# worldlife123/cbench_BaSIC

Hardware: AMD Instinct MI355X
Metric: encode+decode Mpix/s (higher is better)
Workload: dtype f32; 1 GPU; hyperprior codec N=128 M=192 (lossy_graph_scalable_exp_hp), synthetic 3x256x256 images (image i = manual_seed(i), rand), 256 images per GPU per step resident in HBM, compress+decompress incl. bitstream D2H/H2D, 4 concurrent stream workers per GPU (step k on worker k mod W: whole batches, W in flight); images_per_gpu=256, workers=4, rans_waves_per_workgroup=8, batches_in_flight=4, parallelism=image-sharded x1, RCCL all-reduce of metric sums

## Files before the change

### cbench_basic_amd/csrc/conv.hip

```cpp
#include "common.h"

#include <cstdlib>
#include <cstring>
#include <new>
#include <vector>

using namespace basic;

namespace {
thread_local bool g_dynamic_tiles = false;
}
namespace basic {
bool set_dynamic_tiles(bool on)
{
    const bool prev = g_dynamic_tiles;
    g_dynamic_tiles = on;
    return prev;
}
}

namespace {

typedef float f32x16 __attribute__((ext_vector_type(16)));
typedef float f32x4 __attribute__((ext_vector_type(4)));
// ... 337 lines not shown
    if (lane_live && my < g.mh && mx < g.mw && b < g.batch) {
        const int oy = my * g.s_out + g.oy0, ox = mx * g.s_out + g.ox0;
        const int64_t plane = static_cast<int64_t>(g.out_h) * g.out_w;
        float *o = g.out + (static_cast<int64_t>(b) * g.out_ctotal + co_base) * plane + static_cast<int64_t>(oy) * g.out_w + ox;
#pragma unroll
        for (int m = 0; m < MT; ++m)
#pragma unroll
            for (int r = 0; r < 16; ++r) {
                const int co = 32 * m + 8 * (r >> 2) + 4 * khalf + (r & 3);
                if (co < cout_here) {
                    if constexpr (KWB > 0) {
                        f32x2 v2;
                        v2[0] = apply_act(acc[m][r], g.act);
                        v2[1] = apply_act(acc2[m][r], g.act);
                        *reinterpret_cast<f32x2 *>(o + co * plane) = v2;
                    } else {
                        o[co * plane] = apply_act(acc[m][r], g.act);
                    }
                }
            }
    }
}

typedef __bf16 bf16x8 __attribute__((ext_vector_type(8)));
typedef unsigned u32x4 __attribute__((ext_vector_type(4)));

constexpr int kSplitWaves = 8;
constexpr int kSplitThreads = 64 * kSplitWaves;
constexpr int kSplitCK = 16;
constexpr int kSplitStageTaps = 5;
constexpr int kSplitBlockU4 = 4 * 3 * 64;
constexpr int kSplitStageU4 = kSplitStageTaps * kSplitBlockU4;
constexpr int kSplitWSlots = (kSplitStageU4 + kSplitThreads - 1) / kSplitThreads;
static_assert(kSplitWSlots % 2 == 0, "weight stage in two halves");
constexpr size_t kSplitLdsBytes = 2 * kSplitStageU4 * 16 + 2 * 128 * sizeof(float);

__device__ __forceinline__ void split_bf16x3(const float (&x)[8], u32x4 &p0, u32x4 &p1, u32x4 &p2)
{
#pragma unroll
    for (int i = 0; i < 4; ++i) {
        const unsigned a = __float_as_uint(x[2 * i]), b = __float_as_uint(x[2 * i + 1]);
        const unsigned a0 = a & 0xFFFF0000u, b0 = b & 0xFFFF0000u;
        p0[i] = (a >> 16) | b0;
        const unsigned ra = __float_as_uint(x[2 * i] - __uint_as_float(a0)), rb = __float_as_uint(x[2 * i + 1] - __uint_as_float(b0));
        const unsigned a1 = ra & 0xFFFF0000u, b1 = rb & 0xFFFF0000u;
        p1[i] = (ra >> 16) | b1;
        const unsigned sa = __float_as_uint(__uint_as_float(ra) - __uint_as_float(a1)), sb = __float_as_uint(__uint_as_float(rb) - __uint_as_float(b1));
        p2[i] = (sa >> 16) | (sb & 0xFFFF0000u);
    }
}

__device__ __forceinline__ f32x16 mfma_bf16(const u32x4 &a, const u32x4 &b, const f32x16 &c)
{
    return __builtin_amdgcn_mfma_f32_32x32x16_bf16(__builtin_bit_cast(bf16x8, a), __builtin_bit_cast(bf16x8, b), c, 0, 0, 0);
}

constexpr int kSplitPatchPos = 416;
constexpr int kSplitPieceBytes = kSplitPatchPos * 32;
constexpr size_t kSplitLdsPatchBytes = kSplitLdsBytes + 3 * kSplitPieceBytes;
static_assert(kSplitLdsPatchBytes <= 160 * 1024, "patch beside the weight stages");
static_assert(kSplitLdsBytes % 16 == 0, "16-byte aligned patch");
constexpr int kSplitPatchRounds = (2 * kSplitPatchPos + kSplitThreads - 1) / kSplitThreads;

template <int KH, int KW, int KWB, bool PATCH>
__global__ __launch_bounds__(kSplitThreads, 1) void conv_split_bf16_kernel(const TapLaunch g, const u32x4 *wsplit)
{
    constexpr int MT = 4;
    constexpr int kTapsA = KH * KW, kTapsAll = KH * (KW + KWB);
    constexpr int kGroups = kTapsAll / kSplitStageTaps;
    static_assert(kTapsAll % kSplitStageTaps == 0, "taps per channel block must be whole stages");
    static_assert(KWB > 0 && KWB <= KW, "fused phases: second grid inside the first");
    extern __shared__ u32x4 lds_u4[];
    float *chan_const = reinterpret_cast<float *>(lds_u4 + 2 * kSplitStageU4);

    const int tid = threadIdx.x;
    const int lane = tid & 63;
    const int khalf = lane >> 5;
    const int wave = __builtin_amdgcn_readfirstlane(tid >> 6);

    int bid = xcd_tile(blockIdx.x, gridDim.x);
    const int tx_i = bid % g.tiles_x; bid /= g.tiles_x;
    const int ty_i = bid % g.tiles_y; bid /= g.tiles_y;
    const int TB = 1 << g.tb_log, TH = 1 << g.th_log, TW = 1 << g.tw_log;
    const int b0 = bid * TB, my0 = ty_i * TH, mx0 = tx_i * TW;
    struct Pos { int tb, my, mx; };
    auto pos_of = [&](int t) {
        const int qq = (t >> 6) * 32 + (t & 31);
        return Pos{qq >> (g.tw_log + g.th_log), my0 + ((qq >> g.tw_log) & (TH - 1)), mx0 + (qq & (TW - 1))};
    };
    const Pos lp = pos_of(tid);
    const int tb = lp.tb, b = b0 + lp.tb;

    if (tid < 128) {
        chan_const[tid] = g.bias ? g.bias[tid] : 0.f;
        chan_const[128 + tid] = g.beta ? g.beta[tid] : 1.f;
    }

    const int64_t plane = static_cast<int64_t>(g.in_h) * g.in_w;
    const int nimg = (g.batch - b0 < TB) ? g.batch - b0 : TB;
    const __amdgpu_buffer_rsrc_t rsrc = __builtin_amdgcn_make_buffer_rsrc(
        const_cast<float *>(g.in + static_cast<int64_t>(b0) * g.cin * plane), 0, static_cast<int>(nimg * g.cin * plane * 4), 0x00020000);
    const int gy_l = lp.my * g.s_in + g.dymin, gx_l = lp.mx * g.s_in + g.dxmin;
    const int lane_off = static_cast<int>((((static_cast<int64_t>(tb) * g.cin + 8 * khalf) * g.in_h + gy_l) * g.in_w + gx_l) * 4);
    constexpr int kSpanX = KW;
    static_assert(KH * kSpanX <= 32, "one validity bit per tap offset");
    unsigned vmask = 0;
    if (b < g.batch) {
#pragma unroll
        for (int dy = 0; dy < KH; ++dy)
#pragma unroll
            for (int dx = 0; dx < kSpanX; ++dx) {
                const int yy = gy_l + dy, xx = gx_l + dx;
                if (yy >= 0 && yy < g.in_h && xx >= 0 && xx < g.in_w) vmask |= 1u << (dy * kSpanX + dx);
            }
    }
    const int plane_bytes = static_cast<int>(plane * 4);
    auto tap_row = [](int t) { return t < kTapsA ? t / KW : (t - kTapsA) / KWB; };
    auto tap_col = [](int t) { return t < kTapsA ? t % KW : (t - kTapsA) % KWB + (KW - KWB); };
    auto load_b = [&](int cb, int T, float (&d)[8]) __attribute__((always_inline)) {
        const int dy = tap_row(T), dx = tap_col(T);
        const int voff = ((vmask >> (dy * kSpanX + dx)) & 1u) ? lane_off + (dy * g.in_w + dx) * 4 : 0x7FFFFFF0;
        const int soff = cb * kSplitCK * plane_bytes;
#pragma unroll
        for (int j = 0; j < 8; ++j)
            d[j] = __builtin_bit_cast(float, __builtin_amdgcn_raw_buffer_load_b32(rsrc, voff, soff + j * plane_bytes, 0));
    };

    const int ncb = g.cin / kSplitCK;
    constexpr int kHalf = kSplitWSlots / 2;
    u32x4 wst[kHalf];
    auto fetch_w = [&](int s, int h) __attribute__((always_inline)) {
        const u32x4 *src = wsplit + static_cast<int64_t>(s) * kSplitStageU4 + tid;
#pragma unroll
        for (int sl = h * kHalf; sl < (h + 1) * kHalf; ++sl)
            if (sl * kSplitThreads + tid < kSplitStageU4) wst[sl - h * kHalf] = src[sl * kSplitThreads];
    };
    auto store_w = [&](int buf, int h) __attribute__((always_inline)) {
        u32x4 *dst = lds_u4 + buf * kSplitStageU4 + tid;
#pragma unroll
        for (int sl = h * kHalf; sl < (h + 1) * kHalf; ++sl)
            if (sl * kSplitThreads + tid < kSplitStageU4) dst[sl * kSplitThreads] = wst[sl - h * kHalf];
    };

    char *const patch = reinterpret_cast<char *>(lds_u4) + kSplitLdsBytes;
    const int PW = TW + KW - 1, PH = TH + KH - 1, npos = TB * PH * PW;
    int pvoff[kSplitPatchRounds], brow[KH];
    if constexpr (PATCH) {
#pragma unroll
        for (int r = 0; r < kSplitPatchRounds; ++r) {
            const int i = r * kSplitThreads + tid, p = i >> 1, h = i & 1;
            const int prow = p / PW, x = p - prow * PW, img = prow / PH, row = prow - img * PH;
            const int gy = my0 + g.dymin + row, gx = mx0 + g.dxmin + x;
            const bool inside = i < 2 * npos && img < nimg && gy >= 0 && gy < g.in_h && gx >= 0 && gx < g.in_w;
            pvoff[r] = inside ? static_cast<int>((((static_cast<int64_t>(img) * g.cin + 8 * h) * g.in_h + gy) * g.in_w + gx) * 4)
                              : 0x7FFFFFF0;
        }
#pragma unroll
        for (int dy = 0; dy < KH; ++dy) brow[dy] = ((tb * PH + (lp.my - my0) + dy) * PW + (lp.mx - mx0)) * 32 + 16 * khalf;
    }
    float pf[kSplitPatchRounds][8];
    auto fetch_patch = [&](int cb) __attribute__((always_inline)) {
        const int soff = cb * kSplitCK * plane_bytes;
#pragma unroll
        for (int r = 0; r < kSplitPatchRounds; ++r)
#pragma unroll
            for (int j = 0; j < 8; ++j)
                pf[r][j] = __builtin_bit_cast(float, __builtin_amdgcn_raw_buffer_load_b32(rsrc, pvoff[r], soff + j * plane_bytes, 0));
    };
    auto store_patch = [&]() __attribute__((always_inline)) {
#pragma unroll
        for (int r = 0; r < kSplitPatchRounds; ++r)
            if (r * kSplitThreads + tid < 2 * npos) {
                u32x4 q[3];
                split_bf16x3(pf[r], q[0], q[1], q[2]);
#pragma unroll
                for (int pc = 0; pc < 3; ++pc)
                    *reinterpret_cast<u32x4 *>(patch + (r * kSplitThreads + tid) * 16 + pc * kSplitPieceBytes) = q[pc];
            }
    };
    auto read_b = [&](int T, u32x4 (&d)[3]) __attribute__((always_inline)) {
        const char *src = patch + brow[tap_row(T)] + 32 * tap_col(T);
#pragma unroll
        for (int pc = 0; pc < 3; ++pc) d[pc] = *reinterpret_cast<const u32x4 *>(src + pc * kSplitPieceBytes);
    };

    f32x16 acc[MT], acc2[MT];
#pragma unroll
    for (int m = 0; m < MT; ++m)
#pragma unroll
        for (int r = 0; r < 16; ++r) {
            acc[m][r] = 0.f;
            acc2[m][r] = 0.f;
        }

    float xb[8];
    u32x4 bq[2][3];
    if constexpr (PATCH) fetch_patch(0);
    else load_b(0, 0, xb);
    fetch_w(0, 0);
    store_w(0, 0);
    fetch_w(0, 1);
    store_w(0, 1);
    if constexpr (PATCH) store_patch();
    for (int cb = 0; cb < ncb; ++cb) {
#pragma unroll
        for (int gi = 0; gi < kGroups; ++gi) {
            const int s = cb * kGroups + gi;
            __syncthreads();
            const bool more = s + 1 < ncb * kGroups;
            if (more) fetch_w(s + 1, 0);
            __builtin_amdgcn_sched_barrier(0);
            const u32x4 *wl = lds_u4 + (s & 1) * kSplitStageU4 + lane;
#pragma unroll
            for (int tl = 0; tl < kSplitStageTaps; ++tl) {
                const int T = gi * kSplitStageTaps + tl;
                float xn[8];
                u32x4 bd[3];
                if constexpr (PATCH) {
                    if (T == 0) read_b(0, bq[0]);
                } else {
                    if (T + 1 < kTapsAll) load_b(cb, T + 1, xn);
                    else load_b(cb + 1 < ncb ? cb + 1 : cb, 0, xn);
                    __builtin_amdgcn_sched_barrier(0);
                    split_bf16x3(xb, bd[0], bd[1], bd[2]);
                }
                const u32x4 (&bp)[3] = PATCH ? bq[T & 1] : bd;
                f32x16 (&dst)[MT] = T < kTapsA ? acc : acc2;
                u32x4 ap[2][3];
#pragma unroll
                for (int pc = 0; pc < 3; ++pc) ap[0][pc] = wl[(tl * MT * 3 + pc) * 64];
#pragma unroll
                for (int m = 0; m < MT; ++m) {
                    const int cur = m & 1;
                    if (m + 1 < MT) {
#pragma unroll
                        for (int pc = 0; pc < 3; ++pc) ap[cur ^ 1][pc] = wl[((tl * MT + m + 1) * 3 + pc) * 64];
                    } else if constexpr (PATCH) {
                        if (T + 1 < kTapsAll) read_b(T + 1, bq[(T + 1) & 1]);
                    }
                    __builtin_amdgcn_sched_barrier(0);
                    dst[m] = mfma_bf16(ap[cur][2], bp[0], dst[m]);
                    dst[m] = mfma_bf16(ap[cur][1], bp[1], dst[m]);
                    dst[m] = mfma_bf16(ap[cur][0], bp[2], dst[m]);
                    dst[m] = mfma_bf16(ap[cur][1], bp[0], dst[m]);
                    dst[m] = mfma_bf16(ap[cur][0], bp[1], dst[m]);
                    dst[m] = mfma_bf16(ap[cur][0], bp[0], dst[m]);
                    __builtin_amdgcn_sched_barrier(0);
                }
                if constexpr (!PATCH) {
#pragma unroll
                    for (int j = 0; j < 8; ++j) xb[j] = xn[j];
                }
                if (tl == 1 && more) {
                    store_w((s + 1) & 1, 0);
                    fetch_w(s + 1, 1);
                    __builtin_amdgcn_sched_barrier(0);
                }
                if constexpr (PATCH) {
                    if (gi == 0 && tl == 1) {
                        fetch_patch(cb + 1 < ncb ? cb + 1 : cb);
                        __builtin_amdgcn_sched_barrier(0);
                    }
                }
                if (tl == 3 && more) store_w((s + 1) & 1, 1);
            }
        }
        if constexpr (PATCH) {
            if (cb + 1 < ncb) {
                __syncthreads();
                store_patch();
            }
        }
    }

    const int tid_e = wave * 64 + static_cast<int>(__lane_id());
    const int khalf_e = (tid_e >> 5) & 1, col_e = tid_e & 31;
    float *gl = reinterpret_cast<float *>(lds_u4);
    const bool gdn = g.act == BASIC_ACT_GDN || g.act == BASIC_ACT_IGDN;
    auto finish = [&](f32x16 (&acc)[MT]) __attribute__((always_inline)) {
        if (g.bias) {
#pragma unroll
            for (int m = 0; m < MT; ++m)
#pragma unroll
                for (int rq = 0; rq < 4; ++rq) {
                    const f32x4 b4 = *reinterpret_cast<const f32x4 *>(chan_const + 32 * m + 8 * rq + 4 * khalf_e);
#pragma unroll
                    for (int e = 0; e < 4; ++e) acc[m][4 * rq + e] += b4[e];
                }
        }
        if (gdn) {
            f32x16 nrm[MT];
#pragma unroll
            for (int m = 0; m < MT; ++m)
#pragma unroll
                for (int r = 0; r < 16; ++r) nrm[m][r] = 0.f;
#pragma unroll
            for (int st = 0; st < 64; ++st) {
                const int kk = 32 * (st >> 4) + 8 * ((st & 15) >> 2) + (st & 3);
                float gk[4];
                load_a<4>(gl + ((kk + 4 * khalf_e) * 32 + col_e) * 4, gk);
                const float x = acc[st >> 4][st & 15];
                const float bfrag = x * x;
// ... 28 lines not shown

    const Pos ep = pos_of(tid_e);
    const int my = ep.my, mx = ep.mx, be = b0 + ep.tb;
    if (my < g.mh && mx < g.mw && be < g.batch) {
        const int oy = my * g.s_out + g.oy0, ox = mx * g.s_out + g.ox0;
        const int64_t oplane = static_cast<int64_t>(g.out_h) * g.out_w;
        float *o = g.out + (static_cast<int64_t>(be) * g.out_ctotal + g.co_base) * oplane + static_cast<int64_t>(oy) * g.out_w + ox;
#pragma unroll
        for (int m = 0; m < MT; ++m)
#pragma unroll
            for (int r = 0; r < 16; ++r) {
                const int co = 32 * m + 8 * (r >> 2) + 4 * khalf_e + (r & 3);
                if (co < g.cout) {
                    f32x2 v2;
                    v2[0] = apply_act(acc[m][r], g.act);
                    v2[1] = apply_act(acc2[m][r], g.act);
                    *reinterpret_cast<f32x2 *>(o + co * oplane) = v2;
                }
            }
    }
}

template <int KH, bool PATCH>
hipError_t launch_split(const TapLaunch &g, const u32x4 *ws, int blocks, hipStream_t st)
{
    const hipError_t e = ensure_max_lds(reinterpret_cast<const void *>(conv_split_bf16_kernel<KH, 3, 2, PATCH>));
    if (e != hipSuccess) return e;
    hipLaunchKernelGGL((conv_split_bf16_kernel<KH, 3, 2, PATCH>), dim3(blocks), dim3(kSplitThreads),
                       PATCH ? kSplitLdsPatchBytes : kSplitLdsBytes, st, g, ws);
    return hipGetLastError();
}

constexpr int kFirstSlots = 10;

template <bool ROWS>
__global__ __launch_bounds__(512, 1) void conv5x5_cin4_gdn_persistent_kernel(const TapLaunch g, int ntiles, int *sched)
{
    extern __shared__ float lds[];
    constexpr int MT = 4, kCK = ROWS ? 3 : 4, KW = 5, kSteps = ROWS ? 5 * 8 : 25 * 2;
    constexpr int kWFloats = ROWS ? 80 * 32 * 4 : 25 * 4 * 32 * 4;
    constexpr int kGFloats = 128 * 32 * 4;
    float *wl = lds;
    float *gl = lds + kWFloats;
    const int tid = threadIdx.x;
    const int lane = tid & 63;
    const int wave = __builtin_amdgcn_readfirstlane(tid >> 6);
    const int khalf = lane >> 5, col = lane & 31;
    const int TB = 1 << g.tb_log, TH = 1 << g.th_log, TW = 1 << g.tw_log;
    const int chan_stride = g.ph * g.pwp;
    const int patch_elems = TB * kCK * chan_stride;
    const int patch_pad = (patch_elems + 511) / 512 * 512;
    const int n_pslots = patch_pad / 512;
// ... 457 lines not shown
                pr[a][1] = f32x2{mid[0], mid[1]};
                pr[a][2] = f32x2{mid[1], mid[2]};
                pr[a][3] = f32x2{mid[2], mid[3]};
                pr[a][4] = f32x2{mid[3], v5};
            }
            sm_accumulate<STRIPS>(acc, g.wsm + static_cast<int64_t>(c0 + ci) * kSmWRow, pr);
        }
    }
    sm_store<STRIPS>(acc, g, b, my, mx0);
}

struct Phase {
    int ntaps = 0, dymin = 0, dxmin = 0, span_y = 1, span_x = 1;
    int oy0 = 0, ox0 = 0;
    int ck = 2, cin_pad = 0;
    int kh = 0, kw = 0;
    int kwb = 0;
    int waves = 4;
    signed char dy[kMaxTaps], dx[kMaxTaps];
    float *d_wpack = nullptr;
    float *d_wrow = nullptr;
    int64_t split_wstride = 0;
    void *d_wsplit = nullptr;
};

struct Chunk {
    int co0 = 0, cout = 0, coutp = 0, mt = 0;
    int nsplit = 1;
    std::vector<Phase> phases;
    std::vector<Phase> fused;
    float *d_bias = nullptr;
};

}

struct basic_conv_plan {
    int cin = 0, cout = 0, ksize = 0, stride = 1, padding = 0, output_padding = 0, transposed = 0, act = 0;
    int s_in = 1, s_out = 1;
    std::vector<Chunk> chunks;
    std::vector<Chunk> split;
    float *d_gammaT = nullptr, *d_beta = nullptr;
    float *d_wsm = nullptr, *d_bias4 = nullptr;
    int *d_sched = nullptr;
};

extern "C" void basic_conv_plan_destroy(basic_conv_plan *p)
{
    if (!p) return;
    for (auto *list : {&p->chunks, &p->split})
        for (auto &ch : *list) {
            for (auto &ph : ch.phases) {
                if (ph.d_wpack) (void)hipFree(ph.d_wpack);
                if (ph.d_wrow) (void)hipFree(ph.d_wrow);
                if (ph.d_wsplit) (void)hipFree(ph.d_wsplit);
            }
            for (auto &ph : ch.fused) {
                if (ph.d_wpack) (void)hipFree(ph.d_wpack);
                if (ph.d_wsplit) (void)hipFree(ph.d_wsplit);
            }
            if (ch.d_bias) (void)hipFree(ch.d_bias);
        }
    if (p->d_sched) (void)hipFree(p->d_sched);
    if (p->d_wsm) (void)hipFree(p->d_wsm);
    if (p->d_bias4) (void)hipFree(p->d_bias4);
    if (p->d_gammaT) (void)hipFree(p->d_gammaT);
    if (p->d_beta) (void)hipFree(p->d_beta);
    delete p;
}

namespace {

int upload(const std::vector<float> &h, float **d)
{
    BASIC_HIP_TRY(hipMalloc(d, h.size() * sizeof(float)));
    BASIC_HIP_TRY(hipMemcpy(*d, h.data(), h.size() * sizeof(float), hipMemcpyHostToDevice));
    return BASIC_OK;
}

int pack_split(const std::vector<float> &wp, int ck, int ntaps, int cin, void **d)
{
    const int ncb = cin / kSplitCK;
    std::vector<uint16_t> ws(static_cast<size_t>(ncb) * ntaps * kSplitBlockU4 * 8);
    size_t i = 0;
    for (int cb = 0; cb < ncb; ++cb)
        for (int t = 0; t < ntaps; ++t)
            for (int m = 0; m < 4; ++m)
                for (int pc = 0; pc < 3; ++pc)
                    for (int lane = 0; lane < 64; ++lane)
                        for (int j = 0; j < 8; ++j) {
                            const int c = cb * kSplitCK + 8 * (lane >> 5) + j, o = 32 * m + (lane & 31);
                            float rem = wp[((static_cast<size_t>(c / ck) * ntaps + t) * ck + c % ck) * 32 * 4 + (o % 32) * 4 + o / 32];
                            uint32_t u = 0;
                            for (int k = 0; k <= pc; ++k) {
                                std::memcpy(&u, &rem, 4);
                                const uint32_t hi = u & 0xFFFF0000u;
                                float h;
                                std::memcpy(&h, &hi, 4);
                                if (k < pc) rem -= h;
                            }
                            ws[i++] = static_cast<uint16_t>(u >> 16);
                        }
    BASIC_HIP_TRY(hipMalloc(d, ws.size() * sizeof(uint16_t)));
    BASIC_HIP_TRY(hipMemcpy(*d, ws.data(), ws.size() * sizeof(uint16_t), hipMemcpyHostToDevice));
    return BASIC_OK;
}

int build_chunks(basic_conv_plan *p, const float *weight, const float *bias, int cin, int cout, int slice,
                 std::vector<Chunk> *out)
{
    const int ci_n = p->cin, co_n = p->cout, ksize = p->ksize, stride = p->stride, padding = p->padding;
    const bool transposed = p->transposed != 0;
    const int nph = transposed ? stride : 1;
    const int n_chunks = slice ? 1 : (co_n + kMaxCoutPerLaunch - 1) / kMaxCoutPerLaunch;
    const int per_chunk = slice ? co_n : ((co_n + n_chunks - 1) / n_chunks + 31) / 32 * 32;
    const bool gdn = p->act == BASIC_ACT_GDN || p->act == BASIC_ACT_IGDN;
    auto fusable = [](const Phase &a, const Phase &b) {
        return a.ntaps > 0 && b.ntaps > 0 && a.kh == b.kh && a.dymin == b.dymin && b.kw <= a.kw &&
               b.dxmin - a.dxmin == a.kw - b.kw && a.ox0 == 0 && b.ox0 == 1 &&
               ((a.kh == 3 && a.kw == 3 && b.kw == 2) || (a.kh == 2 && a.kw == 3 && b.kw == 2));
    };
    for (int co0 = 0; co0 < co_n; co0 += per_chunk) {
        Chunk ch;
        ch.co0 = co0;
        ch.cout = (co_n - co0 < per_chunk) ? co_n - co0 : per_chunk;
        ch.mt = slice ? slice / 32 : (ch.cout + 31) / 32;
        ch.coutp = ch.mt * 32;
// ... 98 lines not shown
                f.cin_pad = (ci_n + kFusedCK - 1) / kFusedCK * kFusedCK;
                f.d_wpack = nullptr;
                const int mtp = mtile_pitch(ch.mt);
                f.split_wstride = static_cast<int64_t>(f.cin_pad) * f.ntaps * 32 * mtp;
                std::vector<float> wp(static_cast<size_t>(f.split_wstride) * ch.nsplit, 0.f);
                auto tap_weight = [&](int phase_px, int t, int kw_phase, int dymin_p, int dxmin_p, int c, int og) -> float {
                    const int dyv = dymin_p + t / kw_phase, dxv = dxmin_p + t % kw_phase;
                    const int ky = py + padding - dyv * stride, kx = phase_px + padding - dxv * stride;
                    if (ky < 0 || ky >= ksize || kx < 0 || kx >= ksize) return 0.f;
                    return weight[((static_cast<size_t>(c) * cout + og) * ksize + ky) * ksize + kx];
                };
                for (int c = 0; c < ci_n; ++c)
                    for (int t = 0; t < f.ntaps; ++t)
                        for (int o = 0; o < ch.cout; ++o) {
                            const float w = t < a.ntaps ? tap_weight(0, t, a.kw, a.dymin, a.dxmin, c, co0 + o)
                                                        : tap_weight(1, t - a.ntaps, b.kw, b.dymin, b.dxmin, c, co0 + o);
                            const int ol = o % ch.coutp;
                            wp[static_cast<size_t>(o / ch.coutp) * f.split_wstride +
                               (((static_cast<size_t>(c / kFusedCK) * f.ntaps + t) * kFusedCK + (c % kFusedCK)) * 32 + ol % 32) * mtp + ol / 32] = w;
                        }
                wp.resize(wp.size() + kPackTail, 0.f);
                int rcf = upload(wp, &f.d_wpack);
                if (!rcf && !slice && p->act == BASIC_ACT_IGDN && ch.mt == 4 && ch.nsplit == 1 && ci_n % kSplitCK == 0)
                    rcf = pack_split(wp, kFusedCK, f.ntaps, ci_n, &f.d_wsplit);
                fused.push_back(f);
                if (rcf) { ok = false; }
            }
            if (ok) ch.fused = fused;
            else for (auto &f : fused) {
                if (f.d_wpack) (void)hipFree(f.d_wpack);
                if (f.d_wsplit) (void)hipFree(f.d_wsplit);
            }
        }
        std::vector<float> hb(static_cast<size_t>(ch.coutp) * ch.nsplit, 0.f);
        if (bias) std::memcpy(hb.data(), bias + co0, sizeof(float) * ch.cout);
        const int rc = upload(hb, &ch.d_bias);
        out->push_back(ch);
        if (rc) return rc;
    }
    return BASIC_OK;
}

}

extern "C" int basic_conv_plan_create(const float *weight, const float *bias, int cin, int cout, int ksize, int stride,
                                      int padding, int output_padding, int transposed, int activation,
                                      const float *gamma, const float *beta, int cin_active, int cout_active,
                                      basic_conv_plan **out)
{
    BASIC_REQUIRE(weight && out && cin >= 1 && cout >= 1 && ksize >= 1 && ksize <= 5 && stride >= 1 && stride <= 2 &&
                      padding >= 0 && padding <= ksize,
                  "conv_plan_create: unsupported geometry (k<=5, stride<=2)");
    BASIC_REQUIRE(cin_active >= 1 && cin_active <= cin && cout_active >= 1 && cout_active <= cout,
                  "conv_plan_create: active channel slice out of range");
// ... 133 lines not shown
    constexpr int kMany = stage_channels(kMaxTaps, WM), kFew = stage_channels(kFewTaps, WF), kVeryFew = stage_channels(kVeryFewTaps, WV);
    const int inst_ck = g.ntaps > kFewTaps ? kMany : (g.ntaps > kVeryFewTaps ? kFew : kVeryFew);
    BASIC_REQUIRE(inst_ck == plan_ck && plan_waves_ == 4, "conv_forward: plan / kernel instantiation mismatch");
    if (g.ntaps > kFewTaps) {
        if (kh == 5 && kw == 5) return launch_one<MT, kMany, 5, 5, WM>(g, blocks, nsplit, lds_bytes, st);
        return launch_one<MT, kMany, 0, 0, WM>(g, blocks, nsplit, lds_bytes, st);
    }
    if (g.ntaps > kVeryFewTaps) {
        if (kh == 3 && kw == 3) return launch_one<MT, kFew, 3, 3, WF>(g, blocks, nsplit, lds_bytes, st);
        return launch_one<MT, kFew, 0, 0, WF>(g, blocks, nsplit, lds_bytes, st);
    }
    if (kh == 3 && kw == 2) return launch_one<MT, kVeryFew, 3, 2, WV>(g, blocks, nsplit, lds_bytes, st);
    if (kh == 2 && kw == 3) return launch_one<MT, kVeryFew, 2, 3, WV>(g, blocks, nsplit, lds_bytes, st);
    if (kh == 2 && kw == 2) return launch_one<MT, kVeryFew, 2, 2, WV>(g, blocks, nsplit, lds_bytes, st);
    return launch_one<MT, kVeryFew, 0, 0, WV>(g, blocks, nsplit, lds_bytes, st);
}

int ilog2(int v) { int l = 0; while ((1 << (l + 1)) <= v) ++l; return l; }
int pow2_ceil(int v) { int p = 1; while (p < v) p <<= 1; return p; }

}

namespace {
struct LaunchChoice { bool use_split, fuse_ok, bf16x3, split_patch; };
LaunchChoice choose_launches(const basic_conv_plan *p, int batch, int oh, int ow, const void *d_out)
{
    const int64_t pos_blocks = (static_cast<int64_t>(batch) * ((oh + p->s_out - 1) / p->s_out) * ((ow + p->s_out - 1) / p->s_out) + kTilePos - 1) / kTilePos;
    const char *dbg_env = getenv("BASIC_CONV_DEBUG");
    const int dbg = dbg_env ? atoi(dbg_env) : 0;
    LaunchChoice c;
    c.use_split = !p->split.empty() && !(dbg & 8) && (pos_blocks < kSplitBelowBlocks || (dbg & 4));
    c.fuse_ok = ow % 2 == 0 && (reinterpret_cast<uintptr_t>(d_out) & 7) == 0 && !(dbg & 512);
    const char *f32_env = getenv("BASIC_CONV_F32");
    c.bf16x3 = !(f32_env && atoi(f32_env) != 0);
    c.split_patch = !(dbg & 1024);
    return c;
}

template <class F>
int for_each_launch(const basic_conv_plan *p, const LaunchChoice &c, int oh, int ow, F &&fn)
{
    for (const Chunk &ch : (c.use_split ? p->split : p->chunks))
        for (const Phase &ph : ((c.fuse_ok && !ch.fused.empty()) ? ch.fused : ch.phases)) {
            const int mh = (oh - ph.oy0 + p->s_out - 1) / p->s_out, mw = (ow - ph.ox0 + p->s_out - 1) / p->s_out;
            if (mh <= 0 || mw <= 0) continue;
            const int rc = fn(ch, ph, mh, mw);
            if (rc) return rc;
        }
    return BASIC_OK;
}

struct TileShape { int tw, th, tb; };
TileShape tile_shape(int mh, int mw, int tile_pos)
{
    TileShape t;
    t.tw = pow2_ceil(mw); if (t.tw > 16) t.tw = 16;
    t.th = pow2_ceil(mh); if (t.th > tile_pos / t.tw) t.th = tile_pos / t.tw;
// ... 19 lines not shown
    return BASIC_OK;
}
}

extern "C" int basic_conv_plan_launches(const basic_conv_plan *p, int batch, int in_h, int in_w)
{
    int oh = 0, ow = 0;
    if (!p || batch < 1 || basic_conv_plan_out_hw(p, in_h, in_w, &oh, &ow)) return -1;
    if (p->d_wsm) return 1;
    int n = 0;
    for_each_launch(p, choose_launches(p, batch, oh, ow, nullptr), oh, ow, [&](const Chunk &, const Phase &, int, int) { ++n; return BASIC_OK; });
    return n;
}

extern "C" int basic_conv_forward_dev(const basic_conv_plan *p, const float *d_in, int batch, int in_h, int in_w,
                                      float *d_out, void *hip_stream)
{
    BASIC_REQUIRE(p && d_in && d_out && batch >= 1, "conv_forward: bad argument");
    int oh = 0, ow = 0;
    int rc = basic_conv_plan_out_hw(p, in_h, in_w, &oh, &ow);
    if (rc) return rc;
    if (p->d_wsm) return launch_small_deconv(p, d_in, batch, in_h, in_w, d_out, as_stream(hip_stream));
    const LaunchChoice choice = choose_launches(p, batch, oh, ow, d_out);
    return for_each_launch(p, choice, oh, ow, [&](const Chunk &ch, const Phase &ph, int mh, int mw) -> int {
        TapLaunch g{};
        g.in = d_in; g.out = d_out; g.wpack = ph.d_wpack; g.wrow = ph.d_wrow; g.split_wstride = ph.split_wstride; g.bias = ch.d_bias; g.gammaT = p->d_gammaT; g.beta = p->d_beta;
        g.batch = batch; g.cin = p->cin; g.cin_pad = ph.ntaps ? ph.cin_pad : 0; g.cout = ch.cout; g.coutp = ch.coutp; g.out_ctotal = p->cout; g.co_base = ch.co0;
        g.in_h = in_h; g.in_w = in_w; g.out_h = oh; g.out_w = ow;
        g.s_in = p->s_in; g.s_out = p->s_out; g.oy0 = ph.oy0; g.ox0 = ph.ox0;
        g.mh = mh; g.mw = mw;
        g.ntaps = ph.ntaps; g.dymin = ph.dymin; g.dxmin = ph.dxmin;
        std::memcpy(g.dy, ph.dy, sizeof(g.dy));
        std::memcpy(g.dx, ph.dx, sizeof(g.dx));
        g.act = p->act;
        const int kCK = ph.ck;
        if (choice.bf16x3 && ph.d_wsplit) {
            const TileShape ts = tile_shape(g.mh, g.mw, kSplitWaves * 32);
            const int tw = ts.tw, th = ts.th, tb = ts.tb;
            if (static_cast<int64_t>(tb) * p->cin * in_h * in_w * 4 < (1ll << 31)) {
                g.tw_log = ilog2(tw); g.th_log = ilog2(th); g.tb_log = ilog2(tb);
                g.tiles_y = (g.mh + th - 1) / th;
                g.tiles_x = (g.mw + tw - 1) / tw;
                const int blocks = ((batch + tb - 1) / tb) * g.tiles_y * g.tiles_x;
                hipStream_t st = as_stream(hip_stream);
                const u32x4 *ws = static_cast<const u32x4 *>(ph.d_wsplit);
                BASIC_REQUIRE(ph.kw == 3 && ph.kwb == 2 && (ph.kh == 3 || ph.kh == 2), "conv_forward: split-bf16 plan / kernel instantiation mismatch");
                const bool patch = choice.split_patch && g.s_in == 1 && tb * (th + ph.kh - 1) * (tw + ph.kw - 1) <= kSplitPatchPos;
                const hipError_t e = ph.kh == 3 ? (patch ? launch_split<3, true>(g, ws, blocks, st) : launch_split<3, false>(g, ws, blocks, st))
                                                : (patch ? launch_split<2, true>(g, ws, blocks, st) : launch_split<2, false>(g, ws, blocks, st));
                BASIC_HIP_TRY(e);
                return BASIC_OK;
            }
        }
        const int threads = 64 * ph.waves, tile_pos = 32 * ph.waves;
        const TileShape ts = tile_shape(g.mh, g.mw, tile_pos);
        const int tw = ts.tw, th = ts.th;
        int tb = ts.tb;
        const bool first_layer_path = ch.mt == 4 && ch.nsplit == 1 && ph.waves == 8 && ph.kh == 5 && ph.kw == 5 &&
                                      ph.cin_pad == kCK && kCK == 4 && ch.cout == 128 && p->d_gammaT;
        g.ph = (th - 1) * g.s_in + ph.span_y;
        g.pw = (tw - 1) * g.s_in + ph.span_x;
        g.patch4 = (ph.waves == 8 && !first_layer_path && in_w % 4 == 0 && (reinterpret_cast<uintptr_t>(d_in) & 15) == 0) ? 1 : 0;
        g.pwp = g.patch4 ? (g.pw + 3 + 3) / 4 * 4 : (g.pw | 1);
        const int punit = g.patch4 ? 4 : 1;
        const int mtp = mtile_pitch(ch.mt);
        const int wl_floats = g.ntaps * kCK * 32 * mtp, gam_floats = 32 * 32 * mtp;
        const int wl_pad = ((wl_floats > gam_floats ? wl_floats : gam_floats) + 4 * threads - 1) / (4 * threads) * (4 * threads);
        auto patch_slots_needed = [&](int tbv) { return (tbv * kCK * g.ph * g.pwp / punit + threads - 1) / threads; };
        auto lds_need = [&](int tbv) {
            const int patch_pad = ((tbv * kCK * g.ph * g.pwp / punit + 63) & ~63) * punit;
            return sizeof(float) * (2 * static_cast<size_t>(wl_pad + patch_pad) + 32 + 2 * g.coutp);
        };
// ... 58 lines not shown
```

Before: 818.0 Mpix/s.

## Replace bf16x3 split convolution with exponent-scaled fp16x2 split MFMA

The split-precision decoder deconvolution now splits activations and weights into two fp16 pieces instead of three bf16 pieces. That cuts the MFMAs per tile from six to three and shrinks the weight and patch LDS staging by a third. To keep fp16 in range, weights get a per-output-channel power-of-two scale when packed on the host. Activations get a per-image scale taken from a new absmax prepass kernel, and both scales are undone in the epilogue. The cost is an extra read of the input plus a memset, and a single per-plan amax buffer. That buffer is shared across concurrent stream workers and can be reallocated, so there is a race risk. Precision also differs from the three-way bf16 split.

New measurement: 894.2 Mpix/s (median of 6 runs). +9.3%, better.

```diff
diff --git a/cbench_basic_amd/csrc/conv.hip b/cbench_basic_amd/csrc/conv.hip
--- a/cbench_basic_amd/csrc/conv.hip
+++ b/cbench_basic_amd/csrc/conv.hip
@@ -1,5 +1,7 @@
 #include "common.h"
 
+#include <algorithm>
+#include <cmath>
 #include <cstdlib>
 #include <cstring>
 #include <new>
@@ -383,48 +385,76 @@
     }
 }
 
-typedef __bf16 bf16x8 __attribute__((ext_vector_type(8)));
+typedef _Float16 f16x8 __attribute__((ext_vector_type(8)));
+typedef _Float16 f16x2 __attribute__((ext_vector_type(2)));
 typedef unsigned u32x4 __attribute__((ext_vector_type(4)));
+typedef int i32x4 __attribute__((ext_vector_type(4)));
 
 constexpr int kSplitWaves = 8;
 constexpr int kSplitThreads = 64 * kSplitWaves;
 constexpr int kSplitCK = 16;
 constexpr int kSplitStageTaps = 5;
-constexpr int kSplitBlockU4 = 4 * 3 * 64;
+constexpr int kSplitBlockU4 = 4 * 2 * 64;
 constexpr int kSplitStageU4 = kSplitStageTaps * kSplitBlockU4;
 constexpr int kSplitWSlots = (kSplitStageU4 + kSplitThreads - 1) / kSplitThreads;
-static_assert(kSplitWSlots % 2 == 0, "weight stage in two halves");
-constexpr size_t kSplitLdsBytes = 2 * kSplitStageU4 * 16 + 2 * 128 * sizeof(float);
-
-__device__ __forceinline__ void split_bf16x3(const float (&x)[8], u32x4 &p0, u32x4 &p1, u32x4 &p2)
+constexpr size_t kSplitLdsBytes = 2 * kSplitStageU4 * 16 + 3 * 128 * sizeof(float);
+constexpr int kSplitWTop = 13, kSplitXTop = 14;
+
+__device__ __forceinline__ int split_act_exp(unsigned amax_bits)
+{
+    const int e = static_cast<int>(amax_bits >> 23);
+    return (amax_bits == 0 || e >= 255) ? 0 : kSplitXTop + 127 - e;
+}
+
+__device__ __forceinline__ void split_f16x2(const float (&x)[8], int k, u32x4 &p0, u32x4 &p1)
 {
 #pragma unroll
     for (int i = 0; i < 4; ++i) {
-        const unsigned a = __float_as_uint(x[2 * i]), b = __float_as_uint(x[2 * i + 1]);
-        const unsigned a0 = a & 0xFFFF0000u, b0 = b & 0xFFFF0000u;
-        p0[i] = (a >> 16) | b0;
-        const unsigned ra = __float_as_uint(x[2 * i] - __uint_as_float(a0)), rb = __float_as_uint(x[2 * i + 1] - __uint_as_float(b0));
-        const unsigned a1 = ra & 0xFFFF0000u, b1 = rb & 0xFFFF0000u;
-        p1[i] = (ra >> 16) | b1;
-        const unsigned sa = __float_as_uint(__uint_as_float(ra) - __uint_as_float(a1)), sb = __float_as_uint(__uint_as_float(rb) - __uint_as_float(b1));
-        p2[i] = (sa >> 16) | (sb & 0xFFFF0000u);
-    }
-}
-
-__device__ __forceinline__ f32x16 mfma_bf16(const u32x4 &a, const u32x4 &b, const f32x16 &c)
-{
-    return __builtin_amdgcn_mfma_f32_32x32x16_bf16(__builtin_bit_cast(bf16x8, a), __builtin_bit_cast(bf16x8, b), c, 0, 0, 0);
+        f32x2 v;
+        v[0] = __builtin_ldexpf(x[2 * i], k);
+        v[1] = __builtin_ldexpf(x[2 * i + 1], k);
+        const f16x2 h0 = __builtin_convertvector(v, f16x2);
+        const f16x2 h1 = __builtin_convertvector(v - __builtin_convertvector(h0, f32x2), f16x2);
+        p0[i] = __builtin_bit_cast(unsigned, h0);
+        p1[i] = __builtin_bit_cast(unsigned, h1);
+    }
+}
+
+__device__ __forceinline__ f32x16 mfma_f16(const u32x4 &a, const u32x4 &b, const f32x16 &c)
+{
+    return __builtin_amdgcn_mfma_f32_32x32x16_f16(__builtin_bit_cast(f16x8, a), __builtin_bit_cast(f16x8, b), c, 0, 0, 0);
+}
+
+__global__ __launch_bounds__(256) void image_absmax_kernel(const float *x, int64_t n, int per_img, unsigned *amax)
+{
+    const int img = blockIdx.x / per_img, part = blockIdx.x - img * per_img;
+    const float *src = x + img * n;
+    unsigned m = 0;
+    if (((reinterpret_cast<uintptr_t>(src) | static_cast<uintptr_t>(n * 4)) & 15) == 0) {
+        const u32x4 *s4 = reinterpret_cast<const u32x4 *>(src);
+        for (int64_t i = part * 256 + threadIdx.x; i < n / 4; i += per_img * 256) {
+            const u32x4 v = s4[i];
+#pragma unroll
+            for (int e = 0; e < 4; ++e) m = max(m, v[e] & 0x7FFFFFFFu);
+        }
+    } else {
+        for (int64_t i = part * 256 + threadIdx.x; i < n; i += per_img * 256) m = max(m, __float_as_uint(src[i]) & 0x7FFFFFFFu);
+    }
+#pragma unroll
+    for (int off = 32; off > 0; off >>= 1) m = max(m, static_cast<unsigned>(__shfl_xor(static_cast<int>(m), off)));
+    if ((threadIdx.x & 63) == 0 && m) atomicMax(amax + img, m);
 }
 
 constexpr int kSplitPatchPos = 416;
 constexpr int kSplitPieceBytes = kSplitPatchPos * 32;
-constexpr size_t kSplitLdsPatchBytes = kSplitLdsBytes + 3 * kSplitPieceBytes;
+constexpr size_t kSplitLdsPatchBytes = kSplitLdsBytes + 2 * kSplitPieceBytes;
 static_assert(kSplitLdsPatchBytes <= 160 * 1024, "patch beside the weight stages");
 static_assert(kSplitLdsBytes % 16 == 0, "16-byte aligned patch");
 constexpr int kSplitPatchRounds = (2 * kSplitPatchPos + kSplitThreads - 1) / kSplitThreads;
 
 template <int KH, int KW, int KWB, bool PATCH>
-__global__ __launch_bounds__(kSplitThreads, 1) void conv_split_bf16_kernel(const TapLaunch g, const u32x4 *wsplit)
+__global__ __launch_bounds__(kSplitThreads, 1) void conv_split_f16_kernel(const TapLaunch g, const u32x4 *wsplit, const int *kw,
+                                                                          const unsigned *amax)
 {
     constexpr int MT = 4;
     constexpr int kTapsA = KH * KW, kTapsAll = KH * (KW + KWB);
@@ -455,6 +485,7 @@
     if (tid < 128) {
         chan_const[tid] = g.bias ? g.bias[tid] : 0.f;
         chan_const[128 + tid] = g.beta ? g.beta[tid] : 1.f;
+        reinterpret_cast<int *>(chan_const)[256 + tid] = kw[tid];
     }
 
     const int64_t plane = static_cast<int64_t>(g.in_h) * g.in_w;
@@ -487,25 +518,28 @@
             d[j] = __builtin_bit_cast(float, __builtin_amdgcn_raw_buffer_load_b32(rsrc, voff, soff + j * plane_bytes, 0));
     };
 
+    int kx_l = 0;
+    if constexpr (!PATCH) kx_l = b < g.batch ? split_act_exp(amax[b]) : 0;
+
     const int ncb = g.cin / kSplitCK;
-    constexpr int kHalf = kSplitWSlots / 2;
+    constexpr int kHalf = (kSplitWSlots + 1) / 2;
     u32x4 wst[kHalf];
     auto fetch_w = [&](int s, int h) __attribute__((always_inline)) {
         const u32x4 *src = wsplit + static_cast<int64_t>(s) * kSplitStageU4 + tid;
 #pragma unroll
-        for (int sl = h * kHalf; sl < (h + 1) * kHalf; ++sl)
+        for (int sl = h * kHalf; sl < (h + 1) * kHalf && sl < kSplitWSlots; ++sl)
             if (sl * kSplitThreads + tid < kSplitStageU4) wst[sl - h * kHalf] = src[sl * kSplitThreads];
     };
     auto store_w = [&](int buf, int h) __attribute__((always_inline)) {
         u32x4 *dst = lds_u4 + buf * kSplitStageU4 + tid;
 #pragma unroll
-        for (int sl = h * kHalf; sl < (h + 1) * kHalf; ++sl)
+        for (int sl = h * kHalf; sl < (h + 1) * kHalf && sl < kSplitWSlots; ++sl)
             if (sl * kSplitThreads + tid < kSplitStageU4) dst[sl * kSplitThreads] = wst[sl - h * kHalf];
     };
 
     char *const patch = reinterpret_cast<char *>(lds_u4) + kSplitLdsBytes;
     const int PW = TW + KW - 1, PH = TH + KH - 1, npos = TB * PH * PW;
-    int pvoff[kSplitPatchRounds], brow[KH];
+    int pvoff[kSplitPatchRounds], pkx[kSplitPatchRounds], brow[KH];
     if constexpr (PATCH) {
 #pragma unroll
         for (int r = 0; r < kSplitPatchRounds; ++r) {
@@ -515,6 +549,7 @@
             const bool inside = i < 2 * npos && img < nimg && gy >= 0 && gy < g.in_h && gx >= 0 && gx < g.in_w;
             pvoff[r] = inside ? static_cast<int>((((static_cast<int64_t>(img) * g.cin + 8 * h) * g.in_h + gy) * g.in_w + gx) * 4)
                               : 0x7FFFFFF0;
+            pkx[r] = inside ? split_act_exp(amax[b0 + img]) : 0;
         }
 #pragma unroll
         for (int dy = 0; dy < KH; ++dy) brow[dy] = ((tb * PH + (lp.my - my0) + dy) * PW + (lp.mx - mx0)) * 32 + 16 * khalf;
@@ -532,17 +567,17 @@
 #pragma unroll
         for (int r = 0; r < kSplitPatchRounds; ++r)
             if (r * kSplitThreads + tid < 2 * npos) {
-                u32x4 q[3];
-                split_bf16x3(pf[r], q[0], q[1], q[2]);
-#pragma unroll
-                for (int pc = 0; pc < 3; ++pc)
+                u32x4 q[2];
+                split_f16x2(pf[r], pkx[r], q[0], q[1]);
+#pragma unroll
+                for (int pc = 0; pc < 2; ++pc)
                     *reinterpret_cast<u32x4 *>(patch + (r * kSplitThreads + tid) * 16 + pc * kSplitPieceBytes) = q[pc];
             }
     };
-    auto read_b = [&](int T, u32x4 (&d)[3]) __attribute__((always_inline)) {
+    auto read_b = [&](int T, u32x4 (&d)[2]) __attribute__((always_inline)) {
         const char *src = patch + brow[tap_row(T)] + 32 * tap_col(T);
 #pragma unroll
-        for (int pc = 0; pc < 3; ++pc) d[pc] = *reinterpret_cast<const u32x4 *>(src + pc * kSplitPieceBytes);
+        for (int pc = 0; pc < 2; ++pc) d[pc] = *reinterpret_cast<const u32x4 *>(src + pc * kSplitPieceBytes);
     };
 
     f32x16 acc[MT], acc2[MT];
@@ -555,7 +590,7 @@
         }
 
     float xb[8];
-    u32x4 bq[2][3];
+    u32x4 bq[2][2];
     if constexpr (PATCH) fetch_patch(0);
     else load_b(0, 0, xb);
     fetch_w(0, 0);
@@ -576,36 +611,36 @@
             for (int tl = 0; tl < kSplitStageTaps; ++tl) {
                 const int T = gi * kSplitStageTaps + tl;
                 float xn[8];
-                u32x4 bd[3];
+                u32x4 bd[2];
                 if constexpr (PATCH) {
                     if (T == 0) read_b(0, bq[0]);
                 } else {
                     if (T + 1 < kTapsAll) load_b(cb, T + 1, xn);
                     else load_b(cb + 1 < ncb ? cb + 1 : cb, 0, xn);
                     __builtin_amdgcn_sched_barrier(0);
-                    split_bf16x3(xb, bd[0], bd[1], bd[2]);
-                }
-                const u32x4 (&bp)[3] = PATCH ? bq[T & 1] : bd;
+                    split_f16x2(xb, kx_l, bd[0], bd[1]);
+                }
+                const u32x4 (&bp)[2] = PATCH ? bq[T & 1] : bd;
                 f32x16 (&dst)[MT] = T < kTapsA ? acc : acc2;
-                u32x4 ap[2][3];
-#pragma unroll
-                for (int pc = 0; pc < 3; ++pc) ap[0][pc] = wl[(tl * MT * 3 + pc) * 64];
+                u32x4 ap[3][2];
+#pragma unroll
+                for (int mm = 0; mm < 2; ++mm)
+#pragma unroll
+                    for (int pc = 0; pc < 2; ++pc) ap[mm][pc] = wl[((tl * MT + mm) * 2 + pc) * 64];
 #pragma unroll
                 for (int m = 0; m < MT; ++m) {
-                    const int cur = m & 1;
-                    if (m + 1 < MT) {
-#pragma unroll
-                        for (int pc = 0; pc < 3; ++pc) ap[cur ^ 1][pc] = wl[((tl * MT + m + 1) * 3 + pc) * 64];
-                    } else if constexpr (PATCH) {
-                        if (T + 1 < kTapsAll) read_b(T + 1, bq[(T + 1) & 1]);
+                    const int cur = m % 3;
+                    if (m + 2 < MT) {
+#pragma unroll
+                        for (int pc = 0; pc < 2; ++pc) ap[(m + 2) % 3][pc] = wl[((tl * MT + m + 2) * 2 + pc) * 64];
+                    }
+                    if constexpr (PATCH) {
+                        if (m == MT - 3 && T + 1 < kTapsAll) read_b(T + 1, bq[(T + 1) & 1]);
                     }
                     __builtin_amdgcn_sched_barrier(0);
-                    dst[m] = mfma_bf16(ap[cur][2], bp[0], dst[m]);
-                    dst[m] = mfma_bf16(ap[cur][1], bp[1], dst[m]);
-                    dst[m] = mfma_bf16(ap[cur][0], bp[2], dst[m]);
-                    dst[m] = mfma_bf16(ap[cur][1], bp[0], dst[m]);
-                    dst[m] = mfma_bf16(ap[cur][0], bp[1], dst[m]);
-                    dst[m] = mfma_bf16(ap[cur][0], bp[0], dst[m]);
+                    dst[m] = mfma_f16(ap[cur][1], bp[0], dst[m]);
+                    dst[m] = mfma_f16(ap[cur][0], bp[1], dst[m]);
+                    dst[m] = mfma_f16(ap[cur][0], bp[0], dst[m]);
                     __builtin_amdgcn_sched_barrier(0);
                 }
                 if constexpr (!PATCH) {
@@ -638,7 +673,17 @@
     const int khalf_e = (tid_e >> 5) & 1, col_e = tid_e & 31;
     float *gl = reinterpret_cast<float *>(lds_u4);
     const bool gdn = g.act == BASIC_ACT_GDN || g.act == BASIC_ACT_IGDN;
+    const int be_s = b0 + pos_of(tid_e).tb;
+    const int kx_e = be_s < g.batch ? split_act_exp(amax[be_s]) : 0;
     auto finish = [&](f32x16 (&acc)[MT]) __attribute__((always_inline)) {
+#pragma unroll
+        for (int m = 0; m < MT; ++m)
+#pragma unroll
+            for (int rq = 0; rq < 4; ++rq) {
+                const i32x4 k4 = *reinterpret_cast<const i32x4 *>(chan_const + 256 + 32 * m + 8 * rq + 4 * khalf_e);
+#pragma unroll
+                for (int e = 0; e < 4; ++e) acc[m][4 * rq + e] = __builtin_ldexpf(acc[m][4 * rq + e], -(k4[e] + kx_e));
+            }
         if (g.bias) {
 #pragma unroll
             for (int m = 0; m < MT; ++m)
@@ -713,12 +758,12 @@
 }
 
 template <int KH, bool PATCH>
-hipError_t launch_split(const TapLaunch &g, const u32x4 *ws, int blocks, hipStream_t st)
-{
-    const hipError_t e = ensure_max_lds(reinterpret_cast<const void *>(conv_split_bf16_kernel<KH, 3, 2, PATCH>));
+hipError_t launch_split(const TapLaunch &g, const u32x4 *ws, const int *kw, const unsigned *amax, int blocks, hipStream_t st)
+{
+    const hipError_t e = ensure_max_lds(reinterpret_cast<const void *>(conv_split_f16_kernel<KH, 3, 2, PATCH>));
     if (e != hipSuccess) return e;
-    hipLaunchKernelGGL((conv_split_bf16_kernel<KH, 3, 2, PATCH>), dim3(blocks), dim3(kSplitThreads),
-                       PATCH ? kSplitLdsPatchBytes : kSplitLdsBytes, st, g, ws);
+    hipLaunchKernelGGL((conv_split_f16_kernel<KH, 3, 2, PATCH>), dim3(blocks), dim3(kSplitThreads),
+                       PATCH ? kSplitLdsPatchBytes : kSplitLdsBytes, st, g, ws, kw, amax);
     return hipGetLastError();
 }
 
@@ -1222,6 +1267,7 @@
     float *d_wrow = nullptr;
     int64_t split_wstride = 0;
     void *d_wsplit = nullptr;
+    int *d_wsplit_k = nullptr;
 };
 
 struct Chunk {
@@ -1242,6 +1288,8 @@
     float *d_gammaT = nullptr, *d_beta = nullptr;
     float *d_wsm = nullptr, *d_bias4 = nullptr;
     int *d_sched = nullptr;
+    unsigned *d_amax = nullptr;
+    int amax_cap = 0;
 };
 
 extern "C" void basic_conv_plan_destroy(basic_conv_plan *p)
@@ -1253,14 +1301,17 @@
                 if (ph.d_wpack) (void)hipFree(ph.d_wpack);
                 if (ph.d_wrow) (void)hipFree(ph.d_wrow);
                 if (ph.d_wsplit) (void)hipFree(ph.d_wsplit);
+                if (ph.d_wsplit_k) (void)hipFree(ph.d_wsplit_k);
             }
             for (auto &ph : ch.fused) {
                 if (ph.d_wpack) (void)hipFree(ph.d_wpack);
                 if (ph.d_wsplit) (void)hipFree(ph.d_wsplit);
+                if (ph.d_wsplit_k) (void)hipFree(ph.d_wsplit_k);
             }
             if (ch.d_bias) (void)hipFree(ch.d_bias);
         }
     if (p->d_sched) (void)hipFree(p->d_sched);
+    if (p->d_amax) (void)hipFree(p->d_amax);
     if (p->d_wsm) (void)hipFree(p->d_wsm);
     if (p->d_bias4) (void)hipFree(p->d_bias4);
     if (p->d_gammaT) (void)hipFree(p->d_gammaT);
@@ -1277,31 +1328,38 @@
     return BASIC_OK;
 }
 
-int pack_split(const std::vector<float> &wp, int ck, int ntaps, int cin, void **d)
+int pack_split(const std::vector<float> &wp, int ck, int ntaps, int cin, void **d, int **d_kw)
 {
     const int ncb = cin / kSplitCK;
-    std::vector<uint16_t> ws(static_cast<size_t>(ncb) * ntaps * kSplitBlockU4 * 8);
+    auto w_at = [&](int c, int t, int o) { return wp[((static_cast<size_t>(c / ck) * ntaps + t) * ck + c % ck) * 32 * 4 + (o % 32) * 4 + o / 32]; };
+    std::vector<int> kw(128, 0);
+    for (int o = 0; o < 128; ++o) {
+        float m = 0.f;
+        for (int c = 0; c < cin; ++c)
+            for (int t = 0; t < ntaps; ++t) m = std::fmax(m, std::fabs(w_at(c, t, o)));
+        int e = 0;
+        if (m > 0.f && std::isfinite(m)) {
+            (void)std::frexp(m, &e);
+            kw[o] = kSplitWTop - (e - 1);
+        }
+    }
+    std::vector<_Float16> ws(static_cast<size_t>(ncb) * ntaps * kSplitBlockU4 * 8);
     size_t i = 0;
     for (int cb = 0; cb < ncb; ++cb)
         for (int t = 0; t < ntaps; ++t)
             for (int m = 0; m < 4; ++m)
-                for (int pc = 0; pc < 3; ++pc)
+                for (int pc = 0; pc < 2; ++pc)
                     for (int lane = 0; lane < 64; ++lane)
                         for (int j = 0; j < 8; ++j) {
                             const int c = cb * kSplitCK + 8 * (lane >> 5) + j, o = 32 * m + (lane & 31);
-                            float rem = wp[((static_cast<size_t>(c / ck) * ntaps + t) * ck + c % ck) * 32 * 4 + (o % 32) * 4 + o / 32];
-                            uint32_t u = 0;
-                            for (int k = 0; k <= pc; ++k) {
-                                std::memcpy(&u, &rem, 4);
-                                const uint32_t hi = u & 0xFFFF0000u;
-                                float h;
-                                std::memcpy(&h, &hi, 4);
-                                if (k < pc) rem -= h;
-                            }
-                            ws[i++] = static_cast<uint16_t>(u >> 16);
+                            const float w = std::ldexp(w_at(c, t, o), kw[o]);
+                            const _Float16 w0 = static_cast<_Float16>(w);
+                            ws[i++] = pc ? static_cast<_Float16>(w - static_cast<float>(w0)) : w0;
                         }
-    BASIC_HIP_TRY(hipMalloc(d, ws.size() * sizeof(uint16_t)));
-    BASIC_HIP_TRY(hipMemcpy(*d, ws.data(), ws.size() * sizeof(uint16_t), hipMemcpyHostToDevice));
+    BASIC_HIP_TRY(hipMalloc(d, ws.size() * sizeof(_Float16)));
+    BASIC_HIP_TRY(hipMemcpy(*d, ws.data(), ws.size() * sizeof(_Float16), hipMemcpyHostToDevice));
+    BASIC_HIP_TRY(hipMalloc(d_kw, kw.size() * sizeof(int)));
+    BASIC_HIP_TRY(hipMemcpy(*d_kw, kw.data(), kw.size() * sizeof(int), hipMemcpyHostToDevice));
     return BASIC_OK;
 }
 
@@ -1446,7 +1504,7 @@
                 wp.resize(wp.size() + kPackTail, 0.f);
                 int rcf = upload(wp, &f.d_wpack);
                 if (!rcf && !slice && p->act == BASIC_ACT_IGDN && ch.mt == 4 && ch.nsplit == 1 && ci_n % kSplitCK == 0)
-                    rcf = pack_split(wp, kFusedCK, f.ntaps, ci_n, &f.d_wsplit);
+                    rcf = pack_split(wp, kFusedCK, f.ntaps, ci_n, &f.d_wsplit, &f.d_wsplit_k);
                 fused.push_back(f);
                 if (rcf) { ok = false; }
             }
@@ -1454,6 +1512,7 @@
             else for (auto &f : fused) {
                 if (f.d_wpack) (void)hipFree(f.d_wpack);
                 if (f.d_wsplit) (void)hipFree(f.d_wsplit);
+                if (f.d_wsplit_k) (void)hipFree(f.d_wsplit_k);
             }
         }
         std::vector<float> hb(static_cast<size_t>(ch.coutp) * ch.nsplit, 0.f);
@@ -1633,7 +1692,7 @@
 }
 
 namespace {
-struct LaunchChoice { bool use_split, fuse_ok, bf16x3, split_patch; };
+struct LaunchChoice { bool use_split, fuse_ok, split_f16, split_patch; };
 LaunchChoice choose_launches(const basic_conv_plan *p, int batch, int oh, int ow, const void *d_out)
 {
     const int64_t pos_blocks = (static_cast<int64_t>(batch) * ((oh + p->s_out - 1) / p->s_out) * ((ow + p->s_out - 1) / p->s_out) + kTilePos - 1) / kTilePos;
@@ -1643,7 +1702,7 @@
     c.use_split = !p->split.empty() && !(dbg & 8) && (pos_blocks < kSplitBelowBlocks || (dbg & 4));
     c.fuse_ok = ow % 2 == 0 && (reinterpret_cast<uintptr_t>(d_out) & 7) == 0 && !(dbg & 512);
     const char *f32_env = getenv("BASIC_CONV_F32");
-    c.bf16x3 = !(f32_env && atoi(f32_env) != 0);
+    c.split_f16 =!(f32_env && atoi(f32_env) != 0);
     c.split_patch = !(dbg & 1024);
     return c;
 }
@@ -1709,6 +1768,7 @@
     if (rc) return rc;
     if (p->d_wsm) return launch_small_deconv(p, d_in, batch, in_h, in_w, d_out, as_stream(hip_stream));
     const LaunchChoice choice = choose_launches(p, batch, oh, ow, d_out);
+    bool amax_done = false;
     return for_each_launch(p, choice, oh, ow, [&](const Chunk &ch, const Phase &ph, int mh, int mw) -> int {
         TapLaunch g{};
         g.in = d_in; g.out = d_out; g.wpack = ph.d_wpack; g.wrow = ph.d_wrow; g.split_wstride = ph.split_wstride; g.bias = ch.d_bias; g.gammaT = p->d_gammaT; g.beta = p->d_beta;
@@ -1721,7 +1781,7 @@
         std::memcpy(g.dx, ph.dx, sizeof(g.dx));
         g.act = p->act;
         const int kCK = ph.ck;
-        if (choice.bf16x3 && ph.d_wsplit) {
+        if (choice.split_f16 && ph.d_wsplit) {
             const TileShape ts = tile_shape(g.mh, g.mw, kSplitWaves * 32);
             const int tw = ts.tw, th = ts.th, tb = ts.tb;
             if (static_cast<int64_t>(tb) * p->cin * in_h * in_w * 4 < (1ll << 31)) {
@@ -1731,10 +1791,26 @@
                 const int blocks = ((batch + tb - 1) / tb) * g.tiles_y * g.tiles_x;
                 hipStream_t st = as_stream(hip_stream);
                 const u32x4 *ws = static_cast<const u32x4 *>(ph.d_wsplit);
-                BASIC_REQUIRE(ph.kw == 3 && ph.kwb == 2 && (ph.kh == 3 || ph.kh == 2), "conv_forward: split-bf16 plan / kernel instantiation mismatch");
+                BASIC_REQUIRE(ph.kw == 3 && ph.kwb == 2 && (ph.kh == 3 || ph.kh == 2), "conv_forward: split-fp16 plan / kernel instantiation mismatch");
+                if (!amax_done) {
+                    auto *pm = const_cast<basic_conv_plan *>(p);
+                    if (pm->amax_cap < batch) {
+                        if (pm->d_amax) BASIC_HIP_TRY(hipFree(pm->d_amax));
+                        pm->d_amax = nullptr; pm->amax_cap = 0;
+                        BASIC_HIP_TRY(hipMalloc(&pm->d_amax, sizeof(unsigned) * batch));
+                        pm->amax_cap = batch;
+                    }
+                    BASIC_HIP_TRY(hipMemsetAsync(pm->d_amax, 0, sizeof(unsigned) * batch, st));
+                    const int64_t n = static_cast<int64_t>(p->cin) * in_h * in_w;
+                    const int per_img = static_cast<int>(std::min<int64_t>(64, std::max<int64_t>(1, n / 4096)));
+                    hipLaunchKernelGGL(image_absmax_kernel, dim3(batch * per_img), dim3(256), 0, st, d_in, n, per_img, pm->d_amax);
+                    BASIC_HIP_TRY(hipGetLastError());
+                    amax_done = true;
+                }
                 const bool patch = choice.split_patch && g.s_in == 1 && tb * (th + ph.kh - 1) * (tw + ph.kw - 1) <= kSplitPatchPos;
-                const hipError_t e = ph.kh == 3 ? (patch ? launch_split<3, true>(g, ws, blocks, st) : launch_split<3, false>(g, ws, blocks, st))
-                                                : (patch ? launch_split<2, true>(g, ws, blocks, st) : launch_split<2, false>(g, ws, blocks, st));
+                const unsigned *am = p->d_amax;
+                const hipError_t e = ph.kh == 3 ? (patch ? launch_split<3, true>(g, ws, ph.d_wsplit_k, am, blocks, st) : launch_split<3, false>(g, ws, ph.d_wsplit_k, am, blocks, st))
+                                                : (patch ? launch_split<2, true>(g, ws, ph.d_wsplit_k, am, blocks, st) : launch_split<2, false>(g, ws, ph.d_wsplit_k, am, blocks, st));
                 BASIC_HIP_TRY(e);
                 return BASIC_OK;
             }
```
